# bcgsc/ntCard

Hardware: AMD Instinct MI355X
Metric: k-mers/s hashed+sketched (whole node) at k=32, 150 bp reads (higher is better)
Workload: dtype u64

## Files before the change

ntcard_amd/csrc/ntc_apply.hip:

```cpp
#include <hip/hip_runtime.h>
#include <stdint.h>

#include <type_traits>

#include "ntc_kernels.hpp"

namespace ntc {

namespace {

constexpr uint32_t kSplitThreads = 1024;
constexpr uint32_t kSplitKeysMax = 8;

__device__ __forceinline__ uint32_t wave_incl_scan(uint32_t v)
{
	const int lane = threadIdx.x & 63;
	for (int o = 1; o < 64; o <<= 1) {
		const uint32_t t = __shfl_up(v, o);
		if (lane >= o) v += t;
	}
	return v;
}

}

constexpr uint32_t kPackBits = 21;
constexpr uint32_t kPackMask = (1u << kPackBits) - 1u;
__device__ __forceinline__ uint32_t pack_count(unsigned long long w) { return (w >> 63) ? ((w >> 42) & 1ull ? 1u : 2u) : 3u; }

#ifdef NTC_SPLIT_CLOCKS
__device__ unsigned long long g_split_clocks[3 * 1024];
}
extern "C" int ntc_dbg_split_clocks(unsigned long long* out) { return (int)hipMemcpyFromSymbol(out, HIP_SYMBOL(ntc::g_split_clocks), sizeof(unsigned long long) * 3 * 1024); }
namespace ntc {
#endif

template <uint32_t kSplitKeys, bool kPackIn, bool kPackOut>
__device__ __forceinline__ void split_body(const SplitArgs& a)
{
#ifdef NTC_SPLIT_CLOCKS
	const unsigned long long sc_t0 = __builtin_amdgcn_s_memrealtime();
#endif
#ifndef NTC_AB_SPLIT_WORDS_DIV
#define NTC_AB_SPLIT_WORDS_DIV 2
#endif
	constexpr uint32_t kWords = kSplitKeys / NTC_AB_SPLIT_WORDS_DIV;
	constexpr uint32_t kPerThread = kPackIn ? 3u * kWords : kSplitKeys;
	constexpr uint32_t kSplitRound = kSplitThreads * kPerThread;
	constexpr uint32_t kLoads = kPackIn ? kWords : kSplitKeys;
	constexpr uint32_t kLoadRound = kSplitThreads * kLoads;
#ifndef NTC_AB_RUN_CHUNK
#define NTC_AB_RUN_CHUNK 256
#endif
	constexpr uint32_t kRunChunk = NTC_AB_RUN_CHUNK;
	__shared__ uint32_t hist[256], excl[256], rel[256], gcur[256], cntd[kPackOut ? 256 : 1], run_n[kRunChunk], tot[1];
	__shared__ uint32_t sorted[kSplitRound + (kPackOut ? 2 * 256 : 0)];
	const uint32_t tid = threadIdx.x, w = blockIdx.x;
	const uint32_t nb = 1u << a.bits, dmask = nb - 1u;
	constexpr bool pack_out = kPackOut;
	if (tid < 256) {
		gcur[tid] = 0;
		hist[tid] = 0;
	}
	uint32_t seg0, step, n_t, hi = 0;
	if (a.mode == 0) {
		seg0 = 0;
		step = gridDim.x;
		n_t = (a.n_in + step - 1u) / step;
	} else {
		const uint32_t b = w / a.parts, p = w % a.parts;
		seg0 = p * a.nb_in + b;
		step = a.parts * a.nb_in;
		n_t = seg0 < a.n_in ? (a.n_in - seg0 + step - 1u) / step : 0u;
		hi = b << a.hi_shift;
	}
	auto seg_of = [&](uint32_t t) -> uint32_t {
#ifdef NTC_AB_OLD_ORDER
		return a.mode == 0 ? t * step + w : seg0 + t * step;
#else
		return a.mode == 0 ? t * step + (w + t) % step : seg0 + t * step;
#endif
	};
	const bool narrow = a.narrow != 0;
	const uint32_t esz_log = pack_out ? 3u : (narrow ? 1u : 2u);
	unsigned char* const outb = reinterpret_cast<unsigned char*>(a.out) + (((uint64_t)w * nb * a.out_cap) << esz_log);
	using load_t = typename std::conditional<kPackIn, unsigned long long, uint32_t>::type;
	for (uint32_t t0 = 0; t0 < n_t; t0 += kRunChunk) {
		const uint32_t t_end = n_t - t0 < kRunChunk ? n_t : t0 + kRunChunk;
		__syncthreads();
		if (tid < kRunChunk && t0 + tid < t_end) {
			const uint32_t sg = seg_of(t0 + tid);
			const uint32_t n = sg < a.n_in ? a.in_cnt[sg] : 0u;
			run_n[tid] = n < a.in_cap ? n : a.in_cap;
		}
		__syncthreads();
		auto next_run = [&](uint32_t t) -> uint32_t {
			while (t < t_end && run_n[t - t0] == 0u)
				++t;
			return t;
		};
		load_t nxt[kLoads];
		auto fetch = [&](uint32_t t, uint32_t base) {
			const uint32_t n = run_n[t - t0];
			const load_t* src = reinterpret_cast<const load_t*>(a.in) + (uint64_t)seg_of(t) * a.in_cap;
#pragma unroll
			for (int j = 0; j < (int)kLoads; ++j) {
				const uint32_t i = base + (uint32_t)j * kSplitThreads + tid;
				nxt[j] = src[i < n ? i : n - 1u];
			}
		};
		uint32_t t = next_run(t0), base = 0;
		if (t < t_end) fetch(t, 0);
		while (t < t_end) {
			const uint32_t n = run_n[t - t0];
			const uint32_t m_in = n - base < kLoadRound ? n - base : kLoadRound;
			uint32_t tn = t, basen = base + kLoadRound;
			if (basen >= n) {
				tn = next_run(t + 1u);
				basen = 0;
			}
			uint32_t key[kPerThread], rank[kPerThread];
			bool have[kPerThread];
#pragma unroll
			for (int j = 0; j < (int)kLoads; ++j) {
				const uint32_t i = (uint32_t)j * kSplitThreads + tid;
				if constexpr (kPackIn) {
					const unsigned long long wd = nxt[j];
					const uint32_t nv = i < m_in ? pack_count(wd) : 0u;
#pragma unroll
					for (int q = 0; q < 3; ++q) {
						key[3 * j + q] = ((uint32_t)(wd >> (kPackBits * q)) & kPackMask) | hi;
						have[3 * j + q] = (uint32_t)q < nv;
					}
				} else {
					key[j] = (uint32_t)nxt[j];
					have[j] = i < m_in;
				}
			}
#pragma unroll
			for (int j = 0; j < (int)kPerThread; ++j)
				rank[j] = have[j] ? atomicAdd(&hist[(key[j] >> a.shift) & dmask], 1u) : 0u;
			if (tn < t_end) fetch(tn, basen);
			__syncthreads();
			if (tid < 64) {
				uint32_t v[4], q[4];
#pragma unroll
				for (int u = 0; u < 4; ++u) {
					v[u] = hist[4 * tid + u];
					q[u] = pack_out ? (v[u] + 2u) / 3u * 3u : v[u];
				}
				const uint32_t s4 = q[0] + q[1] + q[2] + q[3];
				const uint32_t incl = wave_incl_scan(s4);
				uint32_t b0 = incl - s4;
#pragma unroll
				for (int u = 0; u < 4; ++u) {
					excl[4 * tid + u] = b0;
					rel[4 * tid + u] = gcur[4 * tid + u] - (pack_out ? b0 / 3u : b0);
					if constexpr (kPackOut) cntd[4 * tid + u] = v[u];
					b0 += q[u];
				}
				if (tid == 63) tot[0] = incl;
			}
			__syncthreads();
#pragma unroll
			for (int j = 0; j < (int)kPerThread; ++j)
				if (have[j]) sorted[excl[(key[j] >> a.shift) & dmask] + rank[j]] = key[j];
			if (tid < 256) {
				gcur[tid] += pack_out ? (hist[tid] + 2u) / 3u : hist[tid];
				hist[tid] = 0;
			}
			__syncthreads();
			const uint32_t m = tot[0];
			if constexpr (kPackOut) {
				for (uint32_t j = tid; j < m / 3u; j += kSplitThreads) {
					const uint32_t k0 = sorted[3u * j], k1 = sorted[3u * j + 1u], k2 = sorted[3u * j + 2u];
					const uint32_t d = (k0 >> a.shift) & dmask;
					const uint32_t left = cntd[d] - (3u * j - excl[d]);
					const uint32_t nv = left < 3u ? left : 3u;
					const uint32_t off = rel[d] + j;
					if (off < a.out_cap) {
						unsigned long long wd = (unsigned long long)(k0 & kPackMask);
						if (nv >= 2u) wd |= (unsigned long long)(k1 & kPackMask) << kPackBits;
						if (nv == 3u) wd |= (unsigned long long)(k2 & kPackMask) << (2u * kPackBits);
						else wd |= (1ull << 63) | (nv == 1u ? 1ull << 42 : 0ull);
						reinterpret_cast<unsigned long long*>(outb)[(uint64_t)d * a.out_cap + off] = wd;
					} else {
						atomicAdd(a.sketch + k0, 1u);
						if (nv >= 2u) atomicAdd(a.sketch + k1, 1u);
						if (nv == 3u) atomicAdd(a.sketch + k2, 1u);
						if (a.sk_dirty) *a.sk_dirty = 1u;
					}
				}
			} else {
				for (uint32_t i = tid; i < m; i += kSplitThreads) {
					const uint32_t kk = sorted[i];
					const uint32_t off = rel[(kk >> a.shift) & dmask] + i;
					if (off < a.out_cap) {
						const uint64_t at = (uint64_t)((kk >> a.shift) & dmask) * a.out_cap + off;
						if (narrow) reinterpret_cast<uint16_t*>(outb)[at] = (uint16_t)kk;
						else reinterpret_cast<uint32_t*>(outb)[at] = kk;
					} else {
						atomicAdd(a.sketch + kk, 1u);
						if (a.sk_dirty) *a.sk_dirty = 1u;
					}
				}
			}
			__syncthreads();
			t = tn;
			base = basen;
		}
	}
	__syncthreads();
	if (tid < nb) a.out_cnt[(uint64_t)w * nb + tid] = gcur[tid] < a.out_cap ? gcur[tid] : a.out_cap;
#ifdef NTC_SPLIT_CLOCKS
	if (threadIdx.x == 0 && a.mode == 1 && blockIdx.x < 1024u) {
		g_split_clocks[3 * w] = sc_t0;
		g_split_clocks[3 * w + 1] = __builtin_amdgcn_s_memrealtime();
		g_split_clocks[3 * w + 2] = __builtin_amdgcn_s_getreg((4 << 0) | (0 << 6) | (31 << 11)) | ((unsigned long long)__builtin_amdgcn_s_getreg((20 << 0) | (0 << 6) | (31 << 11)) << 32);
	}
#endif
}

template <uint32_t kSplitKeys, bool kPackOut>
__global__ __launch_bounds__(kSplitThreads) void split_kernel(const SplitArgs a)
{
	split_body<kSplitKeys, false, kPackOut>(a);
}
template <uint32_t kSplitKeys>
__global__ __launch_bounds__(kSplitThreads) __attribute__((amdgpu_num_sgpr(80))) void split_packed_kernel(const SplitArgs a)
{
	split_body<kSplitKeys, true, false>(a);
}

#ifndef NTC_AB_COUNT_LOADS
#define NTC_AB_COUNT_LOADS 8
#endif
constexpr uint32_t kCountLoads = NTC_AB_COUNT_LOADS;
template <bool kIn16>
__global__ __launch_bounds__(1024) void count_kernel(const CountArgs a)
{
	extern __shared__ __align__(16) uint32_t cnt[];
	using key_t = typename std::conditional<kIn16, uint16_t, uint32_t>::type;
	const uint32_t tid = threadIdx.x, nt = blockDim.x;
	typedef const __attribute__((address_space(4))) uint32_t* scalar_ptr;
	const scalar_ptr in_cnt = (scalar_ptr)(uintptr_t)a.in_cnt;
	const uint32_t n_cnt = 1u << a.slice_bits, cmask = n_cnt - 1u, n_words = n_cnt >> 1;
	const bool clean = a.first != 0u && (a.sk_dirty == nullptr || __builtin_amdgcn_readfirstlane((int)*a.sk_dirty) == 0);
	for (uint32_t i = tid; i < n_words / 4; i += nt)
		reinterpret_cast<uint4*>(cnt)[i] = make_uint4(0, 0, 0, 0);
	if (a.clear_fill != nullptr)
		for (uint32_t i = blockIdx.x * nt + tid; i < a.n_clear; i += gridDim.x * nt)
			a.clear_fill[i] = 0u;
	__syncthreads();
	for (uint32_t slice = blockIdx.x; slice < a.n_slices; slice += gridDim.x) {
		bool fresh = clean;
		uint32_t seg_add, seg_mul, seg_cnt;
		if (a.mode == 0) {
			seg_add = 0;
			seg_mul = 1;
			seg_cnt = a.n_in;
		} else if (a.mode == 1) {
			seg_add = slice;
			seg_mul = a.nb1;
			seg_cnt = a.nwg1;
		} else {
			const uint32_t b = slice / a.nb2, d2 = slice % a.nb2;
			seg_add = b * a.parts * a.nb2 + d2;
			seg_mul = a.nb2;
			seg_cnt = a.parts;
		}
		uint32_t* dst = a.sketch + ((uint64_t)slice << a.slice_bits);
		uint32_t t = 0, off = 0;
		while (t < seg_cnt && in_cnt[t * seg_mul + seg_add] == 0u)
			++t;
		while (t < seg_cnt) {
			uint32_t taken = 0;
			while (t < seg_cnt && taken < 65535u) {
				const uint32_t seg = t * seg_mul + seg_add;
				uint32_t n = in_cnt[seg];
				n = n < a.in_cap ? n : a.in_cap;
				const uint32_t take = n - off < 65535u - taken ? n - off : 65535u - taken;
				const key_t* src = reinterpret_cast<const key_t*>(a.in) + (uint64_t)seg * a.in_cap + off;
				for (uint32_t base = 0; base < take; base += nt * kCountLoads) {
					uint32_t kq[kCountLoads];
#pragma unroll
					for (uint32_t j = 0; j < kCountLoads; ++j) {
						const uint32_t i = base + j * nt + tid;
						const uint32_t ic = i < take ? i : take - 1u;
						kq[j] = (uint32_t)src[ic];
					}
#pragma unroll
					for (uint32_t j = 0; j < kCountLoads; ++j) {
						const bool have = base + j * nt + tid < take;
						const uint32_t kk = kq[j] & cmask;
						const uint64_t act = __ballot(have);
						if (act == 0) continue;
						const uint32_t first = (uint32_t)__builtin_amdgcn_readlane((int)kk, __builtin_ctzll(act));
						if (__ballot(have && kk == first) == act) {
							if ((tid & 63u) == (uint32_t)__builtin_ctzll(act)) atomicAdd(&cnt[kk >> 1], (uint32_t)__popcll(act) << ((kk & 1u) * 16u));
						} else if (have) {
							atomicAdd(&cnt[kk >> 1], 1u << ((kk & 1u) * 16u));
						}
					}
				}
				taken += take;
				off += take;
				if (off == n) {
					++t;
					off = 0;
				}
			}
			__syncthreads();
			if (taken != 0) {
				if (fresh) {
					for (uint32_t i0 = tid; i0 < n_words / 2; i0 += nt * 4u) {
						uint2 c[4];
#pragma unroll
						for (uint32_t j = 0; j < 4u; ++j) {
							const uint32_t i = i0 + j * nt;
							c[j] = i < n_words / 2 ? reinterpret_cast<const uint2*>(cnt)[i] : make_uint2(0, 0);
						}
#pragma unroll
						for (uint32_t j = 0; j < 4u; ++j) {
							const uint32_t i = i0 + j * nt;
							if ((c[j].x | c[j].y) != 0u) {
								reinterpret_cast<uint2*>(cnt)[i] = make_uint2(0, 0);
								reinterpret_cast<uint4*>(dst)[i] = make_uint4(c[j].x & 0xffffu, c[j].x >> 16, c[j].y & 0xffffu, c[j].y >> 16);
							}
						}
					}
				} else {
					for (uint32_t i0 = tid; i0 < n_words / 2; i0 += nt * 4u) {
						uint2 c[4];
						uint4 s4[4];
#pragma unroll
						for (uint32_t j = 0; j < 4u; ++j) {
							const uint32_t i = i0 + j * nt;
							c[j] = i < n_words / 2 ? reinterpret_cast<const uint2*>(cnt)[i] : make_uint2(0, 0);
							s4[j] = reinterpret_cast<const uint4*>(dst)[(c[j].x | c[j].y) != 0u ? i : 0u];
						}
#pragma unroll
						for (uint32_t j = 0; j < 4u; ++j) {
							const uint32_t i = i0 + j * nt;
							if ((c[j].x | c[j].y) != 0u) {
								reinterpret_cast<uint2*>(cnt)[i] = make_uint2(0, 0);
								uint4 s = s4[j];
								s.x += c[j].x & 0xffffu;
								s.y += c[j].x >> 16;
								s.z += c[j].y & 0xffffu;
								s.w += c[j].y >> 16;
								reinterpret_cast<uint4*>(dst)[i] = s;
							}
						}
					}
				}
				fresh = false;
			}
			__syncthreads();
		}
	}
}

__global__ __launch_bounds__(256) void log_probe_kernel(const uint32_t* __restrict__ log, const uint32_t* __restrict__ fill, uint32_t region_cap,
                                                        uint32_t n_regions, uint32_t per_region, uint32_t* __restrict__ table, uint32_t table_mask,
                                                        unsigned long long* __restrict__ stats)
{
	uint32_t seen = 0, rep = 0;
	for (uint32_t r = blockIdx.x; r < n_regions; r += gridDim.x) {
		uint32_t n = fill[r];
		n = n < region_cap ? n : region_cap;
		n = n < per_region ? n : per_region;
		for (uint32_t i = threadIdx.x; i < n; i += blockDim.x) {
			const uint32_t key = log[(uint64_t)r * region_cap + i];
			const uint32_t slot = (key * 0x9e3779b1u) >> 8 & table_mask;
			const uint32_t old = atomicCAS(&table[slot], 0u, key + 1u);
			++seen;
			rep += old == key + 1u;
		}
	}
	for (int o = 32; o > 0; o >>= 1) {
		seen += __shfl_xor(seen, o);
		rep += __shfl_xor(rep, o);
	}
	if ((threadIdx.x & 63u) == 0u && seen) {
		atomicAdd(stats, (unsigned long long)seen);
		atomicAdd(stats + 1, (unsigned long long)rep);
	}
}

__global__ void log_decide_kernel(unsigned long long* stats, uint32_t* mode, unsigned long long min_keys)
{
	if (stats[0] >= min_keys && *mode == 0u) *mode = (stats[1] * 100ull > stats[0] && stats[1] * 100ull < 90ull * stats[0]) ? 1u : 0u;
	stats[0] = 0;
	stats[1] = 0;
}

hipError_t launch_log_probe(const uint32_t* log, const uint32_t* fill, uint32_t region_cap, uint32_t n_regions, uint32_t per_region, uint32_t* table,
                            uint32_t table_slots, unsigned long long* stats, uint32_t* mode, hipStream_t st)
{
	hipError_t rc = hipMemsetAsync(table, 0, (size_t)table_slots * 4, st);
	if (rc != hipSuccess) return rc;
	hipLaunchKernelGGL(log_probe_kernel, dim3(n_regions < 1024u ? n_regions : 1024u), dim3(256), 0, st, log, fill, region_cap, n_regions, per_region, table,
	                   table_slots - 1u, stats);
	hipLaunchKernelGGL(log_decide_kernel, dim3(1), dim3(1), 0, st, stats, mode, (unsigned long long)(1u << 16));
	return hipGetLastError();
}


__global__ __launch_bounds__(1024) void log_total_kernel(const uint32_t* __restrict__ fill, uint32_t n_regions, uint32_t* __restrict__ total)
{
	__shared__ uint32_t part[16];
	uint32_t s = 0;
	for (uint32_t r = threadIdx.x; r < n_regions; r += blockDim.x)
		s += fill[r] >> 4;
	for (int o = 32; o > 0; o >>= 1)
		s += __shfl_xor(s, o);
	if ((threadIdx.x & 63u) == 0u) part[threadIdx.x >> 6] = s;
	__syncthreads();
	if (threadIdx.x == 0) {
		uint32_t t = 0;
		for (uint32_t w = 0; w < blockDim.x / 64; ++w)
			t += part[w];
		*total = t;
	}
}
__global__ __launch_bounds__(256) void log_atomics_kernel(const uint32_t* __restrict__ log, uint32_t* __restrict__ fill, uint32_t region_cap,
                                                          uint32_t n_regions, const uint32_t* __restrict__ total16, uint32_t max16, uint32_t* __restrict__ sketch,
                                                          uint32_t* __restrict__ sk_dirty)
{
	if (*total16 > max16) return;
	if (sk_dirty && blockIdx.x == 0 && threadIdx.x == 0) *sk_dirty = 1u;
	for (uint32_t r = blockIdx.x; r < n_regions; r += gridDim.x) {
		uint32_t n = fill[r];
		n = n < region_cap ? n : region_cap;
		for (uint32_t i = threadIdx.x; i < n; i += blockDim.x)
			atomicAdd(sketch + log[(uint64_t)r * region_cap + i], 1u);
		__syncthreads();
		if (threadIdx.x == 0) fill[r] = 0;
	}
}

hipError_t launch_log_atomics(const uint32_t* log, uint32_t* fill, uint32_t region_cap, uint32_t n_regions, uint32_t* total16, uint32_t* sketch, uint32_t* sk_dirty,
                              hipStream_t st)
{
	hipLaunchKernelGGL(log_total_kernel, dim3(1), dim3(1024), 0, st, fill, n_regions, total16);
	hipLaunchKernelGGL(log_atomics_kernel, dim3(n_regions < 4096u ? n_regions : 4096u), dim3(256), 0, st, log, fill, region_cap, n_regions, total16,
	                   (4u << 20) >> 4, sketch, sk_dirty);
	return hipGetLastError();
}

__global__ __launch_bounds__(256) void log_export_kernel(const uint32_t* __restrict__ log, const uint32_t* __restrict__ fill, uint32_t region_cap, uint32_t n_regions,
                                                         uint32_t n_parts, uint32_t keys_per_part, uint32_t* __restrict__ out,
                                                         const unsigned long long* __restrict__ part_off, unsigned long long* __restrict__ cursor)
{
	__shared__ uint32_t cnt[64];
	__shared__ unsigned long long base[64];
	const uint32_t tid = threadIdx.x;
	for (uint32_t r = blockIdx.x; r < n_regions; r += gridDim.x) {
		uint32_t n = fill[r];
		n = n < region_cap ? n : region_cap;
		if (n == 0) continue;
		const uint32_t* src = log + (uint64_t)r * region_cap;
		if (tid < 64) cnt[tid] = 0;
		__syncthreads();
		for (uint32_t i = tid; i < n; i += 256u) {
			const uint32_t o = src[i] / keys_per_part;
			atomicAdd(&cnt[o < n_parts ? o : n_parts - 1u], 1u);
		}
		__syncthreads();
		if (tid < n_parts) {
			base[tid] = cnt[tid] ? atomicAdd(&cursor[tid], (unsigned long long)cnt[tid]) : 0ull;
			cnt[tid] = 0;
		}
		__syncthreads();
		if (out != nullptr)
			for (uint32_t i = tid; i < n; i += 256u) {
				const uint32_t key = src[i];
				uint32_t o = key / keys_per_part;
				o = o < n_parts ? o : n_parts - 1u;
				out[part_off[o] + base[o] + atomicAdd(&cnt[o], 1u)] = key;
			}
		__syncthreads();
	}
}

hipError_t launch_log_export(const uint32_t* log, const uint32_t* fill, uint32_t region_cap, uint32_t n_regions, uint32_t n_parts, uint32_t keys_per_part,
                             uint32_t* out, const unsigned long long* part_off, unsigned long long* cursor, hipStream_t st)
{
	hipLaunchKernelGGL(log_export_kernel, dim3(n_regions < 2048u ? n_regions : 2048u), dim3(256), 0, st, log, fill, region_cap, n_regions, n_parts, keys_per_part, out,
	                   part_off, cursor);
	return hipGetLastError();
}

__global__ void log_set_fill_kernel(uint32_t* __restrict__ fill, uint32_t n_regions, uint32_t region_cap, unsigned long long n_keys)
{
	for (uint32_t r = blockIdx.x * blockDim.x + threadIdx.x; r < n_regions; r += gridDim.x * blockDim.x) {
		const unsigned long long lo = (unsigned long long)r * region_cap;
		fill[r] = n_keys <= lo ? 0u : (n_keys - lo < region_cap ? (uint32_t)(n_keys - lo) : region_cap);
	}
}

hipError_t launch_log_set_fill(uint32_t* fill, uint32_t n_regions, uint32_t region_cap, unsigned long long n_keys, hipStream_t st)
{
	hipLaunchKernelGGL(log_set_fill_kernel, dim3((n_regions + 255u) / 256u), dim3(256), 0, st, fill, n_regions, region_cap, n_keys);
	return hipGetLastError();
}

hipError_t launch_split(const SplitArgs& a, unsigned grid, hipStream_t st)
{
	static_assert(kSplitKeysMax == 8, "two sizes of a round");
	if (a.pack_in) {
		if (a.bits >= 7) hipLaunchKernelGGL(split_packed_kernel<8>, dim3(grid), dim3(kSplitThreads), 0, st, a);
		else hipLaunchKernelGGL(split_packed_kernel<4>, dim3(grid), dim3(kSplitThreads), 0, st, a);
	} else {
		if (a.pack_out) {
			if (a.bits >= 7) hipLaunchKernelGGL((split_kernel<8, true>), dim3(grid), dim3(kSplitThreads), 0, st, a);
			else hipLaunchKernelGGL((split_kernel<4, true>), dim3(grid), dim3(kSplitThreads), 0, st, a);
		} else {
			if (a.bits >= 7) hipLaunchKernelGGL((split_kernel<8, false>), dim3(grid), dim3(kSplitThreads), 0, st, a);
			else hipLaunchKernelGGL((split_kernel<4, false>), dim3(grid), dim3(kSplitThreads), 0, st, a);
		}
	}
	return hipGetLastError();
}

hipError_t launch_count(const CountArgs& a, unsigned grid, hipStream_t st)
{
	const size_t smem = (sizeof(uint32_t) << a.slice_bits) / 2;
	if (a.in16) hipLaunchKernelGGL(count_kernel<true>, dim3(grid), dim3(a.slice_bits >= 15 ? 1024 : 512), smem, st, a);
	else hipLaunchKernelGGL(count_kernel<false>, dim3(grid), dim3(a.slice_bits >= 15 ? 1024 : 512), smem, st, a);
	return hipGetLastError();
}

hipError_t set_apply_smem_limit()
{
	hipError_t rc = hipFuncSetAttribute(reinterpret_cast<const void*>(&count_kernel<true>), hipFuncAttributeMaxDynamicSharedMemorySize, 64 * 1024);
	if (rc == hipSuccess) rc = hipFuncSetAttribute(reinterpret_cast<const void*>(&count_kernel<false>), hipFuncAttributeMaxDynamicSharedMemorySize, 64 * 1024);
	return rc;
}

}
```

Measured before the change: 2470 billion.

## Software-pipeline count kernel loads across segments with double-buffered key fetch

Restructures count_kernel into a fetch/consume loop with two register buffers. The next batch of keys is loaded while the previous batch is counted into shared memory, and a batch can draw keys from several input segments so partial batches at segment boundaries are avoided. It also adds a dense, unconditional flush path for fresh 15-bit slices that writes whole lines without zero checks. The price is more complex state tracking, more registers, and an explicit waitcnt, with some risk of subtle bugs at pass boundaries.

```diff
diff --git a/ntcard_amd/csrc/ntc_apply.hip b/ntcard_amd/csrc/ntc_apply.hip
--- a/ntcard_amd/csrc/ntc_apply.hip
+++ b/ntcard_amd/csrc/ntc_apply.hip
@@ -236,6 +236,11 @@
 #define NTC_AB_COUNT_LOADS 8
 #endif
 constexpr uint32_t kCountLoads = NTC_AB_COUNT_LOADS;
+#ifdef NTC_AB_COUNT_SPARSE_FIRST
+constexpr bool count_whole_lines = false;
+#else
+constexpr bool count_whole_lines = true;
+#endif
 template <bool kIn16>
 __global__ __launch_bounds__(1024) void count_kernel(const CountArgs a)
 {
@@ -252,111 +257,168 @@
 		for (uint32_t i = blockIdx.x * nt + tid; i < a.n_clear; i += gridDim.x * nt)
 			a.clear_fill[i] = 0u;
 	__syncthreads();
-	for (uint32_t slice = blockIdx.x; slice < a.n_slices; slice += gridDim.x) {
-		bool fresh = clean;
-		uint32_t seg_add, seg_mul, seg_cnt;
-		if (a.mode == 0) {
-			seg_add = 0;
-			seg_mul = 1;
-			seg_cnt = a.n_in;
-		} else if (a.mode == 1) {
-			seg_add = slice;
-			seg_mul = a.nb1;
-			seg_cnt = a.nwg1;
+	uint32_t c_slice = blockIdx.x, c_add = 0, c_mul = 1, c_cnt = 0;
+	uint32_t c_t = 0, c_off = 0, c_n = 0;
+	auto skip_empty_runs = [&]() {
+		while (c_t < c_cnt) {
+			const uint32_t n = in_cnt[c_t * c_mul + c_add];
+			c_n = n < a.in_cap ? n : a.in_cap;
+			if (c_n != 0u) break;
+			++c_t;
+		}
+	};
+	auto open_slices = [&]() {
+		for (; c_slice < a.n_slices; c_slice += gridDim.x) {
+			if (a.mode == 0) {
+				c_add = 0;
+				c_mul = 1;
+				c_cnt = a.n_in;
+			} else if (a.mode == 1) {
+				c_add = c_slice;
+				c_mul = a.nb1;
+				c_cnt = a.nwg1;
+			} else {
+				const uint32_t b = c_slice / a.nb2, d2 = c_slice % a.nb2;
+				c_add = b * a.parts * a.nb2 + d2;
+				c_mul = a.nb2;
+				c_cnt = a.parts;
+			}
+			c_t = 0;
+			c_off = 0;
+			skip_empty_runs();
+			if (c_t < c_cnt) break;
+		}
+	};
+	auto fetch = [&](uint32_t(&kq)[kCountLoads], uint32_t budget) -> uint32_t {
+		uint64_t at[kCountLoads];
+#pragma unroll
+		for (uint32_t j = 0; j < kCountLoads; ++j)
+			at[j] = 0;
+		uint32_t m = 0;
+		while (m < budget && c_t < c_cnt) {
+			const uint32_t take = c_n - c_off < budget - m ? c_n - c_off : budget - m;
+			const uint64_t e0 = (uint64_t)(c_t * c_mul + c_add) * a.in_cap + c_off;
+#pragma unroll
+			for (uint32_t j = 0; j < kCountLoads; ++j) {
+				const uint32_t rel = j * nt + tid - m;
+				if (rel < take) at[j] = e0 + rel;
+			}
+			m += take;
+			c_off += take;
+			if (c_off == c_n) {
+				++c_t;
+				c_off = 0;
+				skip_empty_runs();
+			}
+		}
+#pragma unroll
+		for (uint32_t j = 0; j < kCountLoads; ++j)
+			kq[j] = (uint32_t)reinterpret_cast<const key_t*>(a.in)[at[j]];
+		return m;
+	};
+	auto consume = [&](const uint32_t(&kq)[kCountLoads], uint32_t m) {
+#pragma unroll
+		for (uint32_t j = 0; j < kCountLoads; ++j) {
+			const bool have = j * nt + tid < m;
+			const uint32_t kk = kq[j] & cmask;
+			const uint64_t act = __ballot(have);
+			if (act == 0) continue;
+			const uint32_t first = (uint32_t)__builtin_amdgcn_readlane((int)kk, __builtin_ctzll(act));
+			if (__ballot(have && kk == first) == act) {
+				if ((tid & 63u) == (uint32_t)__builtin_ctzll(act)) atomicAdd(&cnt[kk >> 1], (uint32_t)__popcll(act) << ((kk & 1u) * 16u));
+			} else if (have) {
+				atomicAdd(&cnt[kk >> 1], 1u << ((kk & 1u) * 16u));
+			}
+		}
+	};
+	const uint32_t round_keys = nt * kCountLoads;
+	bool first_pass = true;
+	uint32_t taken = 0;
+	auto end_of_pass = [&]() {
+		const uint32_t slice = c_slice;
+		uint32_t* dst = a.sketch + ((uint64_t)slice << a.slice_bits);
+		const bool fresh = clean && first_pass;
+		__syncthreads();
+		if (fresh && count_whole_lines && a.slice_bits == 15u && slice + 1u < a.n_slices) {
+			for (uint32_t i0 = tid; i0 < n_words / 2; i0 += nt * 4u) {
+				uint2 c[4];
+#pragma unroll
+				for (uint32_t j = 0; j < 4u; ++j)
+					c[j] = reinterpret_cast<const uint2*>(cnt)[i0 + j * nt];
+#pragma unroll
+				for (uint32_t j = 0; j < 4u; ++j) {
+					reinterpret_cast<uint2*>(cnt)[i0 + j * nt] = make_uint2(0, 0);
+					reinterpret_cast<uint4*>(dst)[i0 + j * nt] = make_uint4(c[j].x & 0xffffu, c[j].x >> 16, c[j].y & 0xffffu, c[j].y >> 16);
+				}
+			}
+		} else if (fresh) {
+			for (uint32_t i0 = tid; i0 < n_words / 2; i0 += nt * 4u) {
+				uint2 c[4];
+#pragma unroll
+				for (uint32_t j = 0; j < 4u; ++j) {
+					const uint32_t i = i0 + j * nt;
+					c[j] = i < n_words / 2 ? reinterpret_cast<const uint2*>(cnt)[i] : make_uint2(0, 0);
+				}
+#pragma unroll
+				for (uint32_t j = 0; j < 4u; ++j) {
+					const uint32_t i = i0 + j * nt;
+					if ((c[j].x | c[j].y) != 0u) {
+						reinterpret_cast<uint2*>(cnt)[i] = make_uint2(0, 0);
+						reinterpret_cast<uint4*>(dst)[i] = make_uint4(c[j].x & 0xffffu, c[j].x >> 16, c[j].y & 0xffffu, c[j].y >> 16);
+					}
+				}
+			}
 		} else {
-			const uint32_t b = slice / a.nb2, d2 = slice % a.nb2;
-			seg_add = b * a.parts * a.nb2 + d2;
-			seg_mul = a.nb2;
-			seg_cnt = a.parts;
-		}
-		uint32_t* dst = a.sketch + ((uint64_t)slice << a.slice_bits);
-		uint32_t t = 0, off = 0;
-		while (t < seg_cnt && in_cnt[t * seg_mul + seg_add] == 0u)
-			++t;
-		while (t < seg_cnt) {
-			uint32_t taken = 0;
-			while (t < seg_cnt && taken < 65535u) {
-				const uint32_t seg = t * seg_mul + seg_add;
-				uint32_t n = in_cnt[seg];
-				n = n < a.in_cap ? n : a.in_cap;
-				const uint32_t take = n - off < 65535u - taken ? n - off : 65535u - taken;
-				const key_t* src = reinterpret_cast<const key_t*>(a.in) + (uint64_t)seg * a.in_cap + off;
-				for (uint32_t base = 0; base < take; base += nt * kCountLoads) {
-					uint32_t kq[kCountLoads];
-#pragma unroll
-					for (uint32_t j = 0; j < kCountLoads; ++j) {
-						const uint32_t i = base + j * nt + tid;
-						const uint32_t ic = i < take ? i : take - 1u;
-						kq[j] = (uint32_t)src[ic];
+			for (uint32_t i0 = tid; i0 < n_words / 2; i0 += nt * 4u) {
+				uint2 c[4];
+				uint4 s4[4];
+#pragma unroll
+				for (uint32_t j = 0; j < 4u; ++j) {
+					const uint32_t i = i0 + j * nt;
+					c[j] = i < n_words / 2 ? reinterpret_cast<const uint2*>(cnt)[i] : make_uint2(0, 0);
+					s4[j] = reinterpret_cast<const uint4*>(dst)[(c[j].x | c[j].y) != 0u ? i : 0u];
+				}
+#pragma unroll
+				for (uint32_t j = 0; j < 4u; ++j) {
+					const uint32_t i = i0 + j * nt;
+					if ((c[j].x | c[j].y) != 0u) {
+						reinterpret_cast<uint2*>(cnt)[i] = make_uint2(0, 0);
+						uint4 s = s4[j];
+						s.x += c[j].x & 0xffffu;
+						s.y += c[j].x >> 16;
+						s.z += c[j].y & 0xffffu;
+						s.w += c[j].y >> 16;
+						reinterpret_cast<uint4*>(dst)[i] = s;
 					}
-#pragma unroll
-					for (uint32_t j = 0; j < kCountLoads; ++j) {
-						const bool have = base + j * nt + tid < take;
-						const uint32_t kk = kq[j] & cmask;
-						const uint64_t act = __ballot(have);
-						if (act == 0) continue;
-						const uint32_t first = (uint32_t)__builtin_amdgcn_readlane((int)kk, __builtin_ctzll(act));
-						if (__ballot(have && kk == first) == act) {
-							if ((tid & 63u) == (uint32_t)__builtin_ctzll(act)) atomicAdd(&cnt[kk >> 1], (uint32_t)__popcll(act) << ((kk & 1u) * 16u));
-						} else if (have) {
-							atomicAdd(&cnt[kk >> 1], 1u << ((kk & 1u) * 16u));
-						}
-					}
-				}
-				taken += take;
-				off += take;
-				if (off == n) {
-					++t;
-					off = 0;
-				}
-			}
-			__syncthreads();
-			if (taken != 0) {
-				if (fresh) {
-					for (uint32_t i0 = tid; i0 < n_words / 2; i0 += nt * 4u) {
-						uint2 c[4];
-#pragma unroll
-						for (uint32_t j = 0; j < 4u; ++j) {
-							const uint32_t i = i0 + j * nt;
-							c[j] = i < n_words / 2 ? reinterpret_cast<const uint2*>(cnt)[i] : make_uint2(0, 0);
-						}
-#pragma unroll
-						for (uint32_t j = 0; j < 4u; ++j) {
-							const uint32_t i = i0 + j * nt;
-							if ((c[j].x | c[j].y) != 0u) {
-								reinterpret_cast<uint2*>(cnt)[i] = make_uint2(0, 0);
-								reinterpret_cast<uint4*>(dst)[i] = make_uint4(c[j].x & 0xffffu, c[j].x >> 16, c[j].y & 0xffffu, c[j].y >> 16);
-							}
-						}
-					}
-				} else {
-					for (uint32_t i0 = tid; i0 < n_words / 2; i0 += nt * 4u) {
-						uint2 c[4];
-						uint4 s4[4];
-#pragma unroll
-						for (uint32_t j = 0; j < 4u; ++j) {
-							const uint32_t i = i0 + j * nt;
-							c[j] = i < n_words / 2 ? reinterpret_cast<const uint2*>(cnt)[i] : make_uint2(0, 0);
-							s4[j] = reinterpret_cast<const uint4*>(dst)[(c[j].x | c[j].y) != 0u ? i : 0u];
-						}
-#pragma unroll
-						for (uint32_t j = 0; j < 4u; ++j) {
-							const uint32_t i = i0 + j * nt;
-							if ((c[j].x | c[j].y) != 0u) {
-								reinterpret_cast<uint2*>(cnt)[i] = make_uint2(0, 0);
-								uint4 s = s4[j];
-								s.x += c[j].x & 0xffffu;
-								s.y += c[j].x >> 16;
-								s.z += c[j].y & 0xffffu;
-								s.w += c[j].y >> 16;
-								reinterpret_cast<uint4*>(dst)[i] = s;
-							}
-						}
-					}
-				}
-				fresh = false;
-			}
-			__syncthreads();
+				}
+			}
+			__builtin_amdgcn_s_waitcnt(0x0f70);
+		}
+		first_pass = c_t == c_cnt;
+		if (first_pass) {
+			c_slice += gridDim.x;
+			open_slices();
+		}
+		taken = 0;
+		__syncthreads();
+	};
+	uint32_t ka[kCountLoads] = {}, kb[kCountLoads] = {};
+	uint32_t ma = 0, mb = 0;
+	open_slices();
+	for (;;) {
+		mb = fetch(kb, 65535u - taken < round_keys ? 65535u - taken : round_keys);
+		taken += mb;
+		consume(ka, ma);
+		if (mb == 0u) {
+			if (taken == 0u) break;
+			end_of_pass();
+		}
+		ma = fetch(ka, 65535u - taken < round_keys ? 65535u - taken : round_keys);
+		taken += ma;
+		consume(kb, mb);
+		if (ma == 0u) {
+			if (taken == 0u) break;
+			end_of_pass();
 		}
 	}
 }
```

New measurement: 2476 billion (median of 4 runs). About the same (+0.3%).
